# Algolzw/image-restoration-sde

Measured on AMD Instinct MI355X. Metric: restored images/sec at 256x256, 100-step IR-SDE reverse sampler, higher is better.
Workload: dtype f32; 1 GPU; IR-SDE deraining ConditionalUNet nf=64 depth=4, reverse_sde, batch=16/GPU 256x256, T=100 (BASELINE.json configs[1]); compute_dtype=fp32, global_batch=16

## Files before the change

image_restoration_sde_amd/_lib.py:

```python
import ctypes
import os
import subprocess
import threading

_HERE = os.path.dirname(os.path.abspath(__file__))
LIB_PATH = os.environ.get("IRSDE_LIB_PATH") or os.path.join(_HERE, "libirsde_hip.so")
CSRC = os.path.join(_HERE, "csrc")

MODE = {"sde": 0, "ode": 1, "posterior": 2, "dsde_sde": 3, "dsde_ode": 4}
COEF_STRIDE = 12
FLAG_KEEP_ACTIVATIONS = 1
FLAG_NAIVE_CONV = 2
FLAG_NO_WINOGRAD = 4
FLAG_NO_WINOGRAD_F43 = 8
FLAG_UNCOND_FULLATTN = 16
FLAG_BF16 = 32
FLAG_NAF_INTRO_SKIP = 64
FLAG_BF16_ACT = 128
FLAG_NO_FUSED_LN = 256
FLAG_NAF_LENS = 512
FLAG_FP16 = 1024
FLAG_NO_WINOGRAD_FUSED = 2048
FLAG_NO_FUSED_ATTN = 4096
FLAG_NO_NAF_CHAIN = 8192
FLAG_SPLIT_BF16X2 = 16384
FLAG_SPLIT_F16X2 = 32768
FLAG_NAF_STEREO = 65536
FLAG_NAF_UNCOND = 131072
FLAG_UNET_STEREO = 262144
FLAG_F16_ACT = 524288
SAMPLE_GRAPH = 1
SAMPLE_PROFILE = 2

SYMBOLS = [
    "irsde_last_error", "irsde_version", "irsde_create", "irsde_create_nafnet", "irsde_destroy", "irsde_num_weights",
    "irsde_weight_name", "irsde_weight_shape", "irsde_load_weight", "irsde_finalize_weights",
    "irsde_set_schedule", "irsde_unet_forward", "irsde_sample", "irsde_sde_step", "irsde_philox_normal",
    "irsde_get_profile", "irsde_debug_tap", "irsde_work_model", "irsde_debug_conv", "irsde_plan_describe", "irsde_bench_conv", "irsde_op_profile", "irsde_debug_split_gemm", "irsde_bench_naf_chain", "irsde_debug_force_subbatches", "irsde_debug_force_chain_groups", "irsde_debug_scam", "irsde_debug_scam_full",
    "irsde_debug_naf_gate_sca", "irsde_debug_tlsc", "irsde_debug_ln_film", "irsde_debug_naf_lnconv", "irsde_debug_naf_chain", "irsde_debug_naf_chain_split_order",
    "irsde_debug_full_attention16",
    "irsde_eval_metrics", "irsde_tensor2img",
    "irsde_set_lens_info", "irsde_nafnet_set_local_pool", "irsde_create_latent_unet", "irsde_latent_shapes", "irsde_latent_encode", "irsde_latent_decode", "irsde_latent_hidden",
]


class IrsdeLibraryError(RuntimeError):
    pass


class IrsdeError(RuntimeError):
    pass


# ... 55 lines not shown
                                 c.c_int, c.c_int, P, P, c.c_int]
    lib.irsde_sde_step.argtypes = [c.c_int, c.c_int, P, P, P, P, P, c.c_uint64, c.c_uint64, c.c_int, c.c_int,
                                   c.c_int, c.c_int, P]
    lib.irsde_philox_normal.argtypes = [P, c.c_int, c.c_int, c.c_int, c.c_uint64, c.c_uint64, P]
    lib.irsde_get_profile.argtypes = [P, c.POINTER(c.c_double)]
    lib.irsde_debug_tap.argtypes = [P, c.c_char_p, P, c.POINTER(c.c_int64)]
    lib.irsde_work_model.argtypes = [P, c.c_int, c.c_int, c.c_int, c.POINTER(c.c_double)]
    lib.irsde_debug_conv.argtypes = [P, c.c_int, P, c.c_int, c.c_int, c.c_int, c.c_int, c.c_int, P, c.c_int, c.c_int,
                                     c.c_int, c.c_int, c.c_int, P, P, c.c_int, c.c_int, P, P, c.c_int, c.c_int, P]
    lib.irsde_plan_describe.argtypes = [P, c.c_int, c.c_int, c.c_int, c.c_char_p, c.c_int]
    lib.irsde_op_profile.argtypes = [P, c.c_char_p, c.c_int]
    lib.irsde_bench_conv.argtypes = [c.c_int] * 11 + [c.POINTER(c.c_double)]
    lib.irsde_bench_naf_chain.argtypes = [c.c_int] * 4 + [c.POINTER(c.c_double)]
    lib.irsde_debug_force_subbatches.argtypes = [c.c_int]
    lib.irsde_debug_force_chain_groups.argtypes = [c.c_int]
    lib.irsde_debug_scam.argtypes = [P, c.c_int, c.c_int, c.c_int, c.c_int] + [P] * 12 + [P, P]
    lib.irsde_debug_scam_full.argtypes = [P, c.c_int, c.c_int, c.c_int, c.c_int] + [P] * 12 + [P, P]
    lib.irsde_debug_naf_gate_sca.argtypes = [P, c.c_int, c.c_int, c.c_int, c.c_int] + [P] * 8
    lib.irsde_debug_tlsc.argtypes = [P] + [c.c_int] * 6 + [P] * 4
    lib.irsde_debug_ln_film.argtypes = [P, c.c_int64, c.c_int, c.c_int64, P, P, P, c.c_int, P, P]
    lib.irsde_debug_naf_lnconv.argtypes = [c.c_int, P, c.c_int64, c.c_int, c.c_int, c.c_int64, P, P, P, c.c_int, P, P, P, c.c_int, P, P, P, P, P]
    lib.irsde_debug_naf_chain.argtypes = [P, P, c.c_int, c.c_int] + [P] * 16 + [P, c.c_int, c.c_int, P, c.c_int, c.c_int, c.c_int, P]
    lib.irsde_debug_naf_chain_split_order.argtypes = [c.c_int, c.c_int, c.POINTER(c.c_int), c.c_int64]
    lib.irsde_debug_full_attention16.argtypes = [P, c.c_int, c.c_int, P, P]
    lib.irsde_debug_split_gemm.argtypes = [P, P, P, c.c_int, c.c_int, c.c_int, c.c_int, c.c_int, P]
    lib.irsde_eval_metrics.argtypes = [P, P, c.c_int, c.c_int, c.c_int, c.c_int, c.c_int, c.POINTER(c.c_double), P]
    lib.irsde_tensor2img.argtypes = [P, P, c.c_int, c.c_int, c.c_int, c.c_int, P]
    lib.irsde_set_lens_info.argtypes = [P, c.POINTER(c.c_float), c.c_int]
    lib.irsde_nafnet_set_local_pool.argtypes = [P, c.c_int, c.c_int, c.c_int, c.c_int]
    lib.irsde_create_latent_unet.argtypes = [c.POINTER(LatentConfig), c.POINTER(P)]
# ... 51 lines not shown
```

image_restoration_sde_amd/csrc/common.h:

```cpp
#pragma once
#include <hip/hip_runtime.h>
#include <cstdint>
#include <cstdio>
#include <cstdlib>
#include <stdexcept>
#include <string>
#include <vector>

namespace irsde {

struct HipError : std::runtime_error {
    using std::runtime_error::runtime_error;
};
struct HipOutOfMemory : HipError {
    using HipError::HipError;
};

inline int tuning_env_int(const char* name, int dflt) {
    static const bool on = [] { const char* t = getenv("IRSDE_TUNING"); return t && atoi(t) == 1; }();
    if (!on) return dflt;
    const char* v = getenv(name);
    return v ? atoi(v) : dflt;
}

// ... 60 lines not shown
    int v_f16 = 0;
    float v_scale = 1.f;
    int v_pairs = 0;
    const float* M = nullptr;
    int Cout = 0;
    float* out = nullptr;
    int out_stride = 0;
    const float* bias = nullptr;
    const float* film = nullptr;
    int film_bstride = 0;
    int silu = 0;
    const float* res = nullptr;
    int res_stride = 0;
};
void launch_wino_input(const WinoParams& p, hipStream_t s);
struct SplitGemmArgs {
    const unsigned short* a = nullptr;
    const unsigned short* b = nullptr;
    float* out = nullptr;
    long long plA = 0, plB = 0, pA = 0, pB = 0, pO = 0;
    int M = 0, N = 0, K = 0, lda = 0, ldc = 0;
    float out_scale = 1.f;
    int n_inner = 1;
    int nblk_n = 0;
};
void gemm_split_global_init();
int gemm_split_inner(int M, int N, int ncomp);
void launch_gemm_split_pairs(const SplitGemmArgs& a, int ncomp, hipStream_t s, int abl = 0, bool f16 = false);
void launch_split_pairs(const float* in, unsigned short* out, size_t rows, int K, hipStream_t s, bool f16 = false,
                        float scale = 1.0f);
// ... 183 lines not shown
```

image_restoration_sde_amd/csrc/engine.h:

```cpp
#pragma once
#include <algorithm>
#include <cmath>
#include <cstring>
#include <functional>
#include <map>
#include <memory>
#include <mutex>
#include <string>
#include <vector>

#include "../../include/irsde_hip.h"
#include "common.h"

namespace irsde {

constexpr int kWinoFusedMaxCin = 256, kWinoFusedMaxCout = 256;
inline long long wino_fused_min_tiles() { return tuning_env_int("IRSDE_WINO_FUSED_MINT", 4096); }
inline bool wino_fused64_enabled() { return tuning_env_int("IRSDE_WINO_FUSED64", 1) != 0; }
inline bool wino_fused64_pair_enabled() { return tuning_env_int("IRSDE_WINO_FUSED64_PAIR", 1) != 0; }
inline int wino_fused64_max_cin() { return tuning_env_int("IRSDE_WINO_FUSED64_MAXCIN", 512); }
inline int wino_fused64_max_cout() { return tuning_env_int("IRSDE_WINO_FUSED64_MAXCOUT", 512); }
inline long long wino_fused64_min_tiles() { return tuning_env_int("IRSDE_WINO_FUSED64_MINT", 1024); }
inline int wino_fused64t_mode() { return tuning_env_int("IRSDE_WINO_FUSED64T", 1); }
inline bool naf_lnconv_enabled() { return tuning_env_int("IRSDE_NAF_LNCONV", 1) != 0; }
inline int naf_chain_split_mode() { return tuning_env_int("IRSDE_NAF_CHAIN_SPLIT", 0); }

inline int wino_min_c(int tile) {
    return tuning_env_int(tile == 4 ? "IRSDE_WINO4_MINC" : "IRSDE_WINO2_MINC", tile == 4 ? 64 : 256);
}

struct DeviceScope {
    int prev = -1;
    explicit DeviceScope(int dev) {
        if (hipGetDevice(&prev) != hipSuccess) prev = -1;
        if (prev != dev) IRSDE_HIP_CHECK(hipSetDevice(dev));
        else prev = -1;
    }
    ~DeviceScope() {
        if (prev >= 0) (void)hipSetDevice(prev);
    }
// ... 7 lines not shown
    bool loaded = false;
};

struct ConvW {
    float* w = nullptr;
    float* bias = nullptr;
    int Cout = 0, Cin = 0, KH = 1, KW = 1;
    float* wino_u2 = nullptr;
    float* wino_u4 = nullptr;
    float* wino_uf = nullptr;
    float* wino_uf64 = nullptr;
    unsigned short* wino_uf64p = nullptr;
    float wino_uf64p_scale = 1.f;
    unsigned short* wino_up = nullptr;
    float wino_up_scale = 1.f;
};
struct ResW {
    ConvW b1, b2, res;
    bool has_res = false;
    float* mlp_w = nullptr;
    float* mlp_b = nullptr;
    int film_off = 0;
    int Cout = 0;
};
struct ScamW {
    int c = 0;
    float *gl = nullptr, *gr = nullptr;
    ConvW l, r;
    float *beta = nullptr, *gamma = nullptr;
};
// ... 48 lines not shown
    const int Ctot = d.C0 + d.C1;
    const int TH = d.Ho / tile, TW = d.Wo / tile, T = d.B * TH * TW;
    const int ncomp = (tile + 2) * (tile + 2);
    w.in.tile = tile;
    w.in.in0 = d.in0; w.in.in1 = d.in1; w.in.C0 = d.C0; w.in.C1 = d.C1; w.in.Hin = d.Hin; w.in.Win = d.Win;
    w.in.in_shift = d.in_shift; w.in.B = d.B; w.in.TH = TH; w.in.TW = TW; w.in.T = T; w.in.V = V;
    w.out = w.in;
    w.out.M = Mb; w.out.Cout = d.Cout; w.out.out = d.out; w.out.out_stride = d.out_stride; w.out.bias = d.bias;
    w.out.film = d.film; w.out.film_bstride = d.film_bstride; w.out.silu = d.silu; w.out.res = d.res;
    w.out.res_stride = d.res_stride;
    ConvParams& g = w.gemm;
    g.in0 = V; g.C0 = Ctot; g.pix0 = Ctot; g.Hin = 1; g.Win = T; g.w = U; g.Cout = d.Cout;
    g.KH = g.KW = 1; g.stride = 1; g.pad_y = g.pad_x = 0; g.B = 1; g.Ho = 1; g.Wo = T;
    g.out = Mb; g.out_stride = d.Cout; g.zeros = d.zeros;
    g.nz = ncomp; g.z_in = (long long)T * Ctot; g.z_w = (long long)d.Cout * Ctot; g.z_out = (long long)T * d.Cout;
    return w;
}
struct WinoSplitPlan {
    WinoParams in, out;
    SplitGemmArgs gemm;
    int nplanes = 0;
    bool f16 = false;
};
inline WinoSplitPlan make_wino_split(const ConvParams& d, const unsigned short* Us, unsigned short* Vs, float* Mb, int nplanes) {
    const WinoPlan w = make_wino(d, nullptr, nullptr, Mb, 4);
    WinoSplitPlan sp;
    sp.in = w.in; sp.out = w.out; sp.nplanes = nplanes;
    const int Ctot = d.C0 + d.C1;
    const long long T = w.in.T;
    sp.in.Vs = Vs; sp.in.nplanes = nplanes; sp.in.v_plane = 36ll * T * Ctot;
// ... 296 lines not shown
```

image_restoration_sde_amd/csrc/engine_debug.hip:

```cpp
#include "engine.h"
#include "../../include/irsde_hip_debug.h"

using namespace irsde;

namespace irsde {
namespace {

struct Scratch {
    hipStream_t s;
    std::vector<void*> bufs;
    explicit Scratch(hipStream_t s_) : s(s_) {}
    ~Scratch() {
        (void)hipStreamSynchronize(s);
        for (void* p : bufs) (void)hipFree(p);
    }
    Scratch(const Scratch&) = delete;
    Scratch& operator=(const Scratch&) = delete;
    template <class T> T* alloc(size_t n) {
        void* p = nullptr;
        IRSDE_HIP_CHECK(hipMalloc(&p, n * sizeof(T)));
        bufs.push_back(p);
        return static_cast<T*>(p);
    }
    float* upload(const float* host, size_t n) {
// ... 30 lines not shown
    for (int i = 0; i < iters; ++i) run();
    IRSDE_HIP_CHECK(hipEventRecord(ev.e1, s));
    IRSDE_HIP_CHECK(hipStreamSynchronize(s));
    float ms = 0.f;
    IRSDE_HIP_CHECK(hipEventElapsedTime(&ms, ev.e0, ev.e1));
    return ms / iters;
}

struct VariantScope {
    explicit VariantScope(int v) { conv_set_variant(v); }
    ~VariantScope() { conv_set_variant(0); }
};

bool code_in(const std::initializer_list<int>& codes, int c) { return std::find(codes.begin(), codes.end(), c) != codes.end(); }
bool debug_conv_code_known(int c) {
    return code_in({0, 1, 2, 3, 4, 5, 12, 13, 22, 23, 33, 34, 35, 36, 37, 42, 43, 44, 45, 46, 47, 55, 56, 62, 63, 204, 260, 261, 262, 263}, c) ||
           code_in({100, 103, 105, 106, 107, 150, 160, 161, 162, 163, 165, 166, 167, 170, 171, 172, 173}, c);
}
bool bench_conv_variant_known(int v) {
    return code_in({0, 3, 5, 6, 7, 50, 60, 61, 62, 63, 64, 65, 66, 67, 70, 71, 72, 73}, v) ||
           code_in({80, 81, 82, 412, 413, 421, 422, 423, 430, 431, 432, 434, 435, 460, 461, 462, 465, 467, 468, 469, 480, 481, 482}, v) ||
           code_in({2001, 2002, 2004, 4650, 4651, 4652, 4653}, v) ||
           (v >= 83 && v <= 82 + 255) ||
           (v >= 472 && v <= 476);
}

struct ScamHookArgs {
    const float* x;
    float* out;
    const float *norm_l_g, *norm_r_g, *l_proj1_w, *l_proj1_b, *r_proj1_w, *r_proj1_b, *l_proj2_w, *l_proj2_b, *r_proj2_w, *r_proj2_b, *beta, *gamma;
};
// ... 260 lines not shown
        p.Hin = Hin; p.Win = Win; p.in_shift = in_shift;
        p.w = dw; p.Cout = Cout; p.KH = KH; p.KW = KW; p.stride = stride; p.pad_y = pad; p.pad_x = pad;
        p.B = B;
        p.Ho = ((Hin << in_shift) + 2 * pad - KH) / stride + 1;
        p.Wo = ((Win << in_shift) + 2 * pad - KW) / stride + 1;
        p.out = out; p.out_stride = Cout; p.bias = db; p.film = film; p.film_bstride = film_bstride; p.silu = silu;
        p.res = res; p.res_stride = Cout;
        float* dz = mem.alloc<float>(256);
        IRSDE_HIP_CHECK(hipMemset(dz, 0, 1024));
        p.zeros = dz;
        const int wino_tile = (naive == 2 || naive == 12 || naive == 22) ? 2 : (naive == 3 || naive == 13 || naive == 23) ? 4 : 0;
        if (splits > 1 && naive != 1 && !wino_tile) {
            p.splits = splits;
            p.partial = mem.alloc<float>((size_t)splits * B * p.Ho * p.Wo * Cout);
        }
        if (naive == 44 || naive == 45) {
            const bool f16 = naive == 44;
            if (!wino_shape_ok(p, 4) || Cin % 32) throw HipError("debug_conv: shape not eligible for the pair GEMM");
            std::vector<float> U((size_t)36 * Cout * Cin);
            wino_transform_weights(pk.data(), Cout, Cin, U.data(), 4);
            const float us = f16 ? pow2_scale_into_512(U.data(), U.size()) : 1.f;
            const long long T = (long long)B * (p.Ho / 4) * (p.Wo / 4);
            float* dU = mem.upload(U);
            unsigned short* dUp = mem.alloc<unsigned short>(2 * U.size());
            unsigned short* dVp = mem.alloc<unsigned short>((size_t)36 * T * Cin * 2);
            float* dM = mem.alloc<float>((size_t)36 * T * Cout);
            launch_split_pairs(dU, dUp, (size_t)36 * Cout, Cin, s, f16, us);
            const WinoSplitPlan sp = make_wino_pairs(p, dUp, dVp, dM, f16, us);
            launch_wino_input(sp.in, s);
            launch_gemm_split_pairs(sp.gemm, 36, s, 0, f16);
            launch_wino_output(sp.out, s);
// ... 130 lines not shown
        g.a = da; g.b = db; g.out = C;
        g.plA = (long long)na; g.plB = (long long)nb;
        g.pA = (long long)M * K; g.pB = (long long)N * K; g.pO = (long long)M * N;
        g.M = M; g.N = N; g.K = K; g.lda = K; g.ldc = N;
        g.n_inner = gemm_split_inner(M, N, ncomp);
        launch_gemm_split(g, nplanes, ncomp, s);
        IRSDE_HIP_CHECK(hipStreamSynchronize(s));
    });
}

int irsde_debug_force_chain_groups(int g) {
    set_force_chain_groups(g == 1 || g == 2 || g == 4 ? g : 0);
    return IRSDE_OK;
}

int irsde_debug_force_subbatches(int n) {
    set_force_subbatches(n < 0 ? 0 : n);
    return IRSDE_OK;
}

int irsde_bench_naf_chain(int variant, int nblocks, int B, int iters, double* ms_out) {
    return guard([&] {
        if (!ms_out || nblocks < 1 || nblocks > 64 || B < 1 || iters < 1) throw HipError("bench_naf_chain: bad argument");
        const int G = variant == 22 ? 2 : (variant == 24 || variant == 25 || variant == 26) ? 4 : 1;
#ifdef IRSDE_PROBES
        if (variant != 0 && variant != 1 && variant != 11 && G == 1) throw HipError("bench_naf_chain: bad variant");
#else
        if (variant != 0 && variant != 1 && G == 1) throw HipError("bench_naf_chain: variant 11 is a measurement twin (make PROBES=1)");
#endif
        conv_global_init();
// ... 325 lines not shown
```

image_restoration_sde_amd/csrc/engine_plan.hip:

```cpp
#include "engine.h"
#include <atomic>

using namespace irsde;

namespace irsde {

struct Builder {
    irsde_engine* e;
    Plan* pl;
    bool reuse;
    bool naive;
    int film_bstride;
    int b0 = 0;
    const float* film_base() const { return film_of(e, pl) + (size_t)b0 * film_bstride; }
    const float* cam_base() const { return e->cam_cur + (size_t)b0 * e->cam_row; }
    const float* fused_ln_g = nullptr;

    bool act_bf16() const { return (e->cfg.flags & IRSDE_FLAG_BF16_ACT) != 0; }
    bool act_f16() const { return (e->cfg.flags & IRSDE_FLAG_F16_ACT) != 0; }
    Tensor talloc(int B, int H, int W, int C, int force_f32 = 0) {
        Tensor t;
        t.B = B; t.H = H; t.W = W; t.C = C;
        t.bf16 = act_bf16() && !force_f32;
        t.f16 = act_f16() && !force_f32;
// ... 72 lines not shown
        const int Hv = in0.H << in_shift, Wv = in0.W << in_shift;
        p.B = in0.B;
        p.Ho = (Hv + 2 * pad - w.KH) / stride + 1;
        p.Wo = (Wv + 2 * pad - w.KW) / stride + 1;
        const int ostr = out_stride ? out_stride : w.Cout;
        Tensor out = talloc(p.B, p.Ho, p.Wo, ostr, out_stride != 0);
        p.out = out.p; p.out_stride = ostr;
        p.in_bf16 = in0.bf16; p.out_bf16 = out.bf16;
        p.ln_g = fused_ln_g;
        if ((in1 && in1->bf16 != in0.bf16) || (res && res->bf16 != out.bf16)) throw HipError("conv: mixed activation storage types");
        p.bias = w.bias;
        p.film = film; p.film_bstride = film ? film_bstride : 0;
        p.silu = silu;
        if (res) { p.res = res->p; p.res_stride = res->C; }
        if (!naive) {
            if (w.wino_up && wino_shape_ok(p, 4) && push_wino(p, w.wino_u4, 4, w.wino_up, w.wino_up_scale)) return out;
            if (w.wino_uf64p && push_wino_fused(p, reinterpret_cast<const float*>(w.wino_uf64p), true, w.wino_uf64p_scale)) return out;
            if (w.wino_uf64 && push_wino_fused(p, w.wino_uf64, true)) return out;
            if (w.wino_uf && push_wino_fused(p, w.wino_uf, false)) return out;
            if (w.wino_u4 && wino_shape_ok(p, 4) && push_wino(p, w.wino_u4, 4)) return out;
            if (w.wino_u2 && wino_shape_ok(p, 2) && push_wino(p, w.wino_u2, 2)) return out;
        }
        push_conv(p);
        return out;
    }

    bool push_wino_fused(const ConvParams& d, const float* Uf, bool k64, float pair_uscale = 0.f) {
        ConvParams dd = d;
        dd.zeros = e->zeros;
        if (pair_uscale != 0.f) dd.pair_scale = 1.0f / (kWinoFused64PairVScale * pair_uscale);
// ... 36 lines not shown
            const size_t b0 = (size_t)i * dd.B;
            q.in0 = dd.in0 + b0 * dd.Hin * dd.Win * dd.pix0;
            if (dd.in1) q.in1 = dd.in1 + b0 * dd.Hin * dd.Win * dd.pix1;
            q.out = dd.out + b0 * dd.Ho * dd.Wo * dd.out_stride;
            if (dd.res) q.res = dd.res + b0 * dd.Ho * dd.Wo * dd.res_stride;
            if (dd.film && dd.film_bstride) q.film = dd.film + b0 * dd.film_bstride;
            slices.push_back(q);
        }
        if (use_t)
            op.fn = [slices, Uf](hipStream_t s) { for (const auto& q : slices) launch_wino_fused64t(q, Uf, s, 0); };
        else if (k64)
            op.fn = [slices, Uf, pair](hipStream_t s) { for (const auto& q : slices) launch_wino_fused64(q, Uf, s, pair ? 4 : 0); };
        else
            op.fn = [slices, Uf](hipStream_t s) { for (const auto& q : slices) launch_wino_fused(q, Uf, s); };
        push_op(std::move(op));
        return true;
    }

    bool push_wino(const ConvParams& d, const float* U, int tile, const unsigned short* Up = nullptr, float up_scale = 1.f) {
        const int Ctot = d.C0 + d.C1;
        const int ncomp = (tile + 2) * (tile + 2);
        const long long T = (long long)d.B * (d.Ho / tile) * (d.Wo / tile);
        const long long gemm_blocks = ncomp * ((T + 127) / 128) * ((d.Cout + 127) / 128);
        if (gemm_blocks < 256) return false;
        ConvParams dd = d;
        dd.zeros = e->zeros;
        if (Up && (T < 256 || d.Cout < 256 || (unsigned long long)T * Ctot * 4ull >= 0xffffffffull)) return false;
        float* V = pl->alloc((size_t)ncomp * T * Ctot, true);
        float* Mb = pl->alloc((size_t)ncomp * T * d.Cout, true);
        WinoPlan wp = make_wino(dd, U, V, Mb, tile);
// ... 646 lines not shown
    if (stereo) {
        float* pred = pl->alloc((size_t)pl->B * pl->Hp * pl->Wp * pl->pred_stride, false);
        const float* src = pr.p;
        const int Bp = pl->B, ic = e->naf_ic, Hp = pl->Hp, Wp = pl->Wp, is = oe.out_stride, os = pl->pred_stride;
        b.push_other(OP_OTHER, [=](hipStream_t s) { launch_stereo_pack_pred(src, pred, Bp, ic, Hp, Wp, is, os, s); });
        pl->net_ops.back().desc = "stereo_pack_pred";
        pl->pred = pred;
        return;
    }
    pl->pred = pr.p;
}

static std::atomic<int> g_force_chain_groups{0};
void set_force_chain_groups(int g) { g_force_chain_groups.store(g, std::memory_order_relaxed); }
int forced_chain_groups() { return g_force_chain_groups.load(std::memory_order_relaxed); }
static std::atomic<int> g_force_subbatches{0};
void set_force_subbatches(int n) { g_force_subbatches.store(n, std::memory_order_relaxed); }
int naf_subbatches(const irsde_engine* e, int B, int H, int W) {
    if (e->arch == 2 || stereo_engine(e) || (e->cfg.flags & (IRSDE_FLAG_NAIVE_CONV | IRSDE_FLAG_KEEP_ACTIVATIONS))) return 1;
    int n = g_force_subbatches.load(std::memory_order_relaxed);
    if (n <= 0) {
        static const int env = tuning_env_int("IRSDE_SUBBATCHES", 0);
        n = env;
    }
    if (n <= 0 && e->arch != 1) n = 1;
    if (n <= 0) {
        bool chain = false;
        const int nlev = (int)e->naf_enc.size(), ps = 1 << nlev;
        const int Hp = (H + ps - 1) / ps * ps, Wp = (W + ps - 1) / ps * ps;
        if ((e->cfg.flags & IRSDE_FLAG_FP16) && !(e->cfg.flags & (IRSDE_FLAG_NO_NAF_CHAIN | IRSDE_FLAG_F16_ACT)))
// ... 298 lines not shown
```

image_restoration_sde_amd/csrc/engine_weights.hip:

```cpp
#include "engine.h"
#include <cmath>

using namespace irsde;

namespace irsde {

void finalize_common(irsde_engine* e);
void add_w(irsde_engine* e, const std::string& name, std::vector<int64_t> shape) {
    e->names.push_back(name);
    HostTensor t;
    t.shape = std::move(shape);
    e->host[name] = std::move(t);
}
void inv_resblock(irsde_engine* e, const std::string& p, int ci, int co) {
    const int td = e->time_dim;
    add_w(e, p + "mlp.1.weight", {2 * co, td});
    add_w(e, p + "mlp.1.bias", {2 * co});
    add_w(e, p + "block1.proj.weight", {co, ci, 3, 3});
    add_w(e, p + "block2.proj.weight", {co, co, 3, 3});
    if (ci != co) add_w(e, p + "res_conv.weight", {co, ci, 1, 1});
}
void inv_attn(irsde_engine* e, const std::string& p, int c) {
    add_w(e, p + "fn.norm.g", {1, c, 1, 1});
    add_w(e, p + "fn.fn.to_qkv.weight", {384, c, 1, 1});
// ... 60 lines not shown
    } else {
        inv_attn(e, "mid_attn.", mid);
    }
    inv_resblock(e, "mid_block2.", mid, mid);
    inv_resblock(e, "final_res_block.", 2 * nf, nf);
    add_w(e, "final_conv.weight", {vout, nf, 3, 3});
    add_w(e, "final_conv.bias", {vout});
}

const HostTensor& need(irsde_engine* e, const std::string& n) {
    auto it = e->host.find(n);
    if (it == e->host.end() || !it->second.loaded) throw HipError("missing weight: " + n);
    return it->second;
}

ConvW pack_conv(irsde_engine* e, const std::string& wname, const std::string& bname) {
    const HostTensor& t = need(e, wname);
    const int O = (int)t.shape[0], I = (int)t.shape[1], KH = (int)t.shape[2], KW = (int)t.shape[3];
    std::vector<float> p((size_t)O * KH * KW * I);
    for (int o = 0; o < O; ++o)
        for (int i = 0; i < I; ++i)
            for (int ky = 0; ky < KH; ++ky)
                for (int kx = 0; kx < KW; ++kx)
                    p[(((size_t)o * KH + ky) * KW + kx) * I + i] = t.data[(((size_t)o * I + i) * KH + ky) * KW + kx];
    ConvW c;
    c.w = e->upload(p);
    c.Cout = O; c.Cin = I; c.KH = KH; c.KW = KW;
    if (!bname.empty()) c.bias = e->upload(need(e, bname).data);
    if (KH == 3 && KW == 3 && I % 32 == 0 && !(e->cfg.flags & (IRSDE_FLAG_NO_WINOGRAD | IRSDE_FLAG_BF16))) {
        for (int tile : {2, 4}) {
            if (tile == 4 && (e->cfg.flags & IRSDE_FLAG_NO_WINOGRAD_F43)) continue;
            if (I < wino_min_c(tile) || O < wino_min_c(tile)) continue;
            std::vector<float> U((size_t)(tile + 2) * (tile + 2) * O * I);
            wino_transform_weights(p.data(), O, I, U.data(), tile);
            (tile == 4 ? c.wino_u4 : c.wino_u2) = e->upload(U);
            if (tile == 4 && (e->cfg.flags & (IRSDE_FLAG_SPLIT_BF16X2 | IRSDE_FLAG_SPLIT_F16X2)) && I >= split_min_cin()) {
                unsigned short* up = nullptr;
                IRSDE_HIP_CHECK(hipMalloc(&up, U.size() * 4));
                e->dev_allocs.push_back(reinterpret_cast<float*>(up));
                const bool f16 = (e->cfg.flags & IRSDE_FLAG_SPLIT_F16X2) != 0;
                if (f16) c.wino_up_scale = pow2_scale_into_512(U.data(), U.size());
                launch_split_pairs(c.wino_u4, up, (size_t)36 * O, I, e->stream, f16, c.wino_up_scale);
                IRSDE_HIP_CHECK(hipStreamSynchronize(e->stream));
// ... 563 lines not shown
        a.qkv = pack_conv(e, "mid_attn.fn.fn.to_qkv.weight", "");
        a.out = pack_conv(e, "mid_attn.fn.fn.to_out.weight", "mid_attn.fn.fn.to_out.bias");
        a.C = a.out.Cout;
        e->mid_attn = a;
    } else {
        e->mid_attn = pack_attn(e, "mid_attn.");
    }
    e->mid2 = pack_res(e, "mid_block2.");
    for (int j = 0; j < depth; ++j) {
        const std::string u = "ups." + std::to_string(j) + ".";
        e->up_res.push_back(pack_res(e, u + "0."));
        e->up_res.push_back(pack_res(e, u + "1."));
        e->up_attn.push_back(pack_attn(e, u + "2."));
        if (stereo) e->up_scam.push_back(pack_scam(e, u + "3."));
        if (j != depth - 1)
            e->up_conv.push_back(pack_conv(e, u + ci + ".1.weight", u + ci + ".1.bias"));
        else
            e->up_conv.push_back(pack_conv(e, u + ci + ".weight", ""));
    }
    e->final_res = pack_res(e, "final_res_block.");
    e->final_conv = pack_conv(e, "final_conv.weight", "final_conv.bias");

    e->all_res.clear();
    for (auto& r : e->down_res) e->all_res.push_back(&r);
    e->all_res.push_back(&e->mid1);
    e->all_res.push_back(&e->mid2);
    for (auto& r : e->up_res) e->all_res.push_back(&r);
    e->all_res.push_back(&e->final_res);
    int off = 0;
    for (ResW* r : e->all_res) {
        r->film_off = off;
// ... 67 lines not shown
```

image_restoration_sde_amd/csrc/wino.hip:

```cpp
#include "common.h"

namespace irsde {
namespace {

__device__ __forceinline__ float4 operator+(float4 a, float4 b) { return make_float4(a.x + b.x, a.y + b.y, a.z + b.z, a.w + b.w); }
__device__ __forceinline__ float4 operator-(float4 a, float4 b) { return make_float4(a.x - b.x, a.y - b.y, a.z - b.z, a.w - b.w); }
__device__ __forceinline__ float4 operator*(float s, float4 a) { return make_float4(s * a.x, s * a.y, s * a.z, s * a.w); }
__device__ __forceinline__ float silu1(float v) { return v / (1.0f + expf(-v)); }
template <typename V> struct VecOps;
template <> struct VecOps<float4> {
    static constexpr int N = 4;
    static __device__ __forceinline__ float4 zero() { return make_float4(0.f, 0.f, 0.f, 0.f); }
    static __device__ __forceinline__ float4 one() { return make_float4(1.f, 1.f, 1.f, 1.f); }
    static __device__ __forceinline__ float4 mad(float4 v, float4 a, float4 b) { return make_float4(v.x * a.x + b.x, v.y * a.y + b.y, v.z * a.z + b.z, v.w * a.w + b.w); }
    static __device__ __forceinline__ float4 silu(float4 v) { return make_float4(silu1(v.x), silu1(v.y), silu1(v.z), silu1(v.w)); }
};
template <> struct VecOps<float> {
    static constexpr int N = 1;
    static __device__ __forceinline__ float zero() { return 0.f; }
    static __device__ __forceinline__ float one() { return 1.f; }
    static __device__ __forceinline__ float mad(float v, float a, float b) { return v * a + b; }
    static __device__ __forceinline__ float silu(float v) { return silu1(v); }
};

// ... 221 lines not shown
    for (int i = 0; i < TILE; ++i) {
        V y[TILE];
        at_apply<TILE, V>(u[i], y);
#pragma unroll
        for (int j = 0; j < TILE; ++j) {
            const size_t pixel = ((size_t)b * Ho + TILE * ty + i) * Wo + TILE * tx + j;
            V v = y[j] + bias;
            if (p.film) v = VecOps<V>::mad(v, sc, sh);
            if (p.silu) v = VecOps<V>::silu(v);
            if (p.res) v = v + *reinterpret_cast<const V*>(p.res + pixel * p.res_stride + n);
            *reinterpret_cast<V*>(p.out + pixel * p.out_stride + n) = v;
        }
    }
}

}

static int wino_vec() {
    static const int v = tuning_env_int("IRSDE_WINO_VEC", 4);
    return v;
}

void launch_wino_input(const WinoParams& p, hipStream_t s) {
    if (p.Vs) {
        if (p.tile != 4 || (p.nplanes != 2 && p.nplanes != 3) || (p.C0 % 4) || (p.C1 % 4)) throw HipError("wino_input (split): F(4x4,3x3), 2 or 3 planes");
        const long long tot = (long long)p.T * ((p.C0 + p.C1) / 4);
        const dim3 gr((unsigned)((tot + 255) / 256));
        if (p.v_pairs) {
            if (p.nplanes != 2 || (p.C0 + p.C1) % 32) throw HipError("wino_input (pairs): two planes, channels a multiple of 32");
            if (p.v_f16) hipLaunchKernelGGL((wino_input_split_kernel<2, true, true>), gr, dim3(256), 0, s, p);
// ... 58 lines not shown
```

include/irsde_hip.h:

```cpp
#ifndef IRSDE_HIP_H
#define IRSDE_HIP_H

#include <stdint.h>

#ifdef __cplusplus
extern "C" {
#endif

typedef struct irsde_engine irsde_engine;

enum {
    IRSDE_OK = 0,
    IRSDE_ERR_INVALID = -1,
    IRSDE_ERR_HIP = -2,
    IRSDE_ERR_STATE = -3,
    IRSDE_ERR_WEIGHT = -4
};

enum { IRSDE_MODE_SDE = 0, IRSDE_MODE_ODE = 1, IRSDE_MODE_POSTERIOR = 2,
       IRSDE_MODE_DSDE_SDE = 3, IRSDE_MODE_DSDE_ODE = 4 };

enum {
    IRSDE_FLAG_KEEP_ACTIVATIONS = 1,
    IRSDE_FLAG_NAIVE_CONV = 2,
// ... 2 lines not shown
    IRSDE_FLAG_BF16 = 32,
    IRSDE_FLAG_BF16_ACT = 128,
    IRSDE_FLAG_NO_FUSED_LN = 256,
    IRSDE_FLAG_NAF_LENS = 512,
    IRSDE_FLAG_NAF_INTRO_SKIP = 64,
    IRSDE_FLAG_FP16 = 1024,
    IRSDE_FLAG_NO_WINOGRAD_FUSED = 2048,
    IRSDE_FLAG_NO_FUSED_ATTN = 4096,
    IRSDE_FLAG_SPLIT_BF16X2 = 16384,
    IRSDE_FLAG_SPLIT_F16X2 = 32768,
    IRSDE_FLAG_NO_NAF_CHAIN = 8192,
    IRSDE_FLAG_NAF_STEREO = 65536,
    IRSDE_FLAG_NAF_UNCOND = 131072,
    IRSDE_FLAG_UNET_STEREO = 262144,
    IRSDE_FLAG_F16_ACT = 524288,
    IRSDE_FLAG_NO_WINOGRAD_F43 = 8
};
enum {
    IRSDE_SAMPLE_GRAPH = 1,
    IRSDE_SAMPLE_PROFILE = 2
};

typedef struct irsde_config {
    int32_t in_nc;
    int32_t out_nc;
    int32_t nf;
    int32_t depth;
    int32_t device;
    int32_t flags;
} irsde_config;
// ... 87 lines not shown
```

include/irsde_hip_debug.h:

```cpp
#ifndef IRSDE_HIP_DEBUG_H
#define IRSDE_HIP_DEBUG_H

#include "irsde_hip.h"

#ifdef __cplusplus
extern "C" {
#endif

int irsde_debug_conv(const float* in0, int C0, const float* in1, int C1, int B, int Hin, int Win, int in_shift,
                     const float* w_oihw, int Cout, int KH, int KW, int stride, int pad, const float* bias,
                     const float* film, int film_bstride, int silu, const float* res, float* out, int naive,
                     int splits, void* stream);

int irsde_debug_split_gemm(const float* A, const float* B, float* C, int M, int N, int K, int ncomp, int nplanes, void* stream);

int irsde_bench_conv(int variant, int B, int H, int W, int Cin, int Cout, int K, int stride, int up, int epi, int iters,
                     double* ms_out);
int irsde_bench_naf_chain(int variant, int nblocks, int B, int iters, double* ms_out);
int irsde_debug_force_subbatches(int n);
int irsde_debug_force_chain_groups(int g);

int irsde_debug_scam(const float* x, int B_pairs, int H, int W, int C, const float* norm_l_g, const float* norm_r_g, const float* l_proj1_w,
                     const float* l_proj1_b, const float* r_proj1_w, const float* r_proj1_b, const float* l_proj2_w, const float* l_proj2_b,
                     const float* r_proj2_w, const float* r_proj2_b, const float* beta, const float* gamma, float* out, void* stream);

int irsde_debug_naf_gate_sca(const float* u, int B, int H, int W, int c, const float* conv2_w, const float* conv2_b, const float* sca_w, const float* sca_b,
                             float* gated_out, float* mean_out, float* s_out, void* stream);
int irsde_debug_tlsc(const float* g, int B, int h, int w, int c, int k1, int k2, float* pooled_out, const float* scale_map, float* scaled_out, void* stream);
int irsde_debug_ln_film(const float* x, long long M, int C, long long ppi, const float* g, const float* fscale, const float* fshift, int film_bstride,
                        float* out, void* stream);
int irsde_debug_naf_lnconv(int mode, const float* x, long long M, int c, int Cout, long long ppi, const float* g, const float* fscale, const float* fshift,
                           int film_bstride, const float* w, const float* bias, const float* gate_film, int gate_film_bstride, const float* in_scale,
                           const float* ch_scale, const float* res, float* out, void* stream);

int irsde_debug_naf_chain(const float* x, float* out, int B, int nblocks, const float* norm1_g, const float* conv1_w, const float* conv1_b, const float* conv2_w,
// ... 16 lines not shown
```

Measured before the change: 4.262 images/s.

## Add polyphase Winograd F(4,2) path for strided-down and upsample convolutions

Adds a Winograd F(4x4,2x2) path that splits 4x4 stride-2 downsampling convs and nearest-upsample-plus-3x3 convs into four 2x2 polyphase sub-kernels. Each is computed through 5x5 input and output transforms around a batched per-component GEMM. The goal is to cut multiply count and direct-conv cost for resampling layers. It is enabled by default behind size heuristics (enough GEMM blocks and FLOPs; upsample only when Cin>=512), with a flag and env/debug overrides to disable it. It adds extra workspace buffers and precomputed transformed weights, and larger Winograd tiles bring some fp32 rounding risk.

```diff
diff --git a/image_restoration_sde_amd/_lib.py b/image_restoration_sde_amd/_lib.py
--- a/image_restoration_sde_amd/_lib.py
+++ b/image_restoration_sde_amd/_lib.py
@@ -29,6 +29,7 @@
 FLAG_NAF_UNCOND = 131072
 FLAG_UNET_STEREO = 262144
 FLAG_F16_ACT = 524288
+FLAG_NO_WINO_POLY = 1048576
 SAMPLE_GRAPH = 1
 SAMPLE_PROFILE = 2
 
@@ -36,7 +37,7 @@
     "irsde_last_error", "irsde_version", "irsde_create", "irsde_create_nafnet", "irsde_destroy", "irsde_num_weights",
     "irsde_weight_name", "irsde_weight_shape", "irsde_load_weight", "irsde_finalize_weights",
     "irsde_set_schedule", "irsde_unet_forward", "irsde_sample", "irsde_sde_step", "irsde_philox_normal",
-    "irsde_get_profile", "irsde_debug_tap", "irsde_work_model", "irsde_debug_conv", "irsde_plan_describe", "irsde_bench_conv", "irsde_op_profile", "irsde_debug_split_gemm", "irsde_bench_naf_chain", "irsde_debug_force_subbatches", "irsde_debug_force_chain_groups", "irsde_debug_scam", "irsde_debug_scam_full",
+    "irsde_get_profile", "irsde_debug_tap", "irsde_work_model", "irsde_debug_conv", "irsde_plan_describe", "irsde_bench_conv", "irsde_op_profile", "irsde_debug_split_gemm", "irsde_bench_naf_chain", "irsde_debug_force_subbatches", "irsde_debug_force_chain_groups", "irsde_debug_force_wino_poly", "irsde_debug_scam", "irsde_debug_scam_full",
     "irsde_debug_naf_gate_sca", "irsde_debug_tlsc", "irsde_debug_ln_film", "irsde_debug_naf_lnconv", "irsde_debug_naf_chain", "irsde_debug_naf_chain_split_order",
     "irsde_debug_full_attention16",
     "irsde_eval_metrics", "irsde_tensor2img",
@@ -122,6 +123,7 @@
     lib.irsde_bench_naf_chain.argtypes = [c.c_int] * 4 + [c.POINTER(c.c_double)]
     lib.irsde_debug_force_subbatches.argtypes = [c.c_int]
     lib.irsde_debug_force_chain_groups.argtypes = [c.c_int]
+    lib.irsde_debug_force_wino_poly.argtypes = [c.c_int]
     lib.irsde_debug_scam.argtypes = [P, c.c_int, c.c_int, c.c_int, c.c_int] + [P] * 12 + [P, P]
     lib.irsde_debug_scam_full.argtypes = [P, c.c_int, c.c_int, c.c_int, c.c_int] + [P] * 12 + [P, P]
     lib.irsde_debug_naf_gate_sca.argtypes = [P, c.c_int, c.c_int, c.c_int, c.c_int] + [P] * 8
diff --git a/image_restoration_sde_amd/csrc/common.h b/image_restoration_sde_amd/csrc/common.h
--- a/image_restoration_sde_amd/csrc/common.h
+++ b/image_restoration_sde_amd/csrc/common.h
@@ -98,6 +98,21 @@
     int res_stride = 0;
 };
 void launch_wino_input(const WinoParams& p, hipStream_t s);
+struct WinoPolyParams {
+    int up = 0;
+    const float* in = nullptr;
+    int C = 0, Hin = 0, Win = 0;
+    int B = 0, TH = 0, TW = 0, T = 0;
+    float* V = nullptr;
+    const float* M = nullptr;
+    int Cout = 0, Ho = 0, Wo = 0;
+    float* out = nullptr;
+    int out_stride = 0;
+    const float* bias = nullptr;
+};
+void launch_wino_poly_input(const WinoPolyParams& p, hipStream_t s);
+void launch_wino_poly_output(const WinoPolyParams& p, hipStream_t s);
+void wino_poly_transform_weights(const float* w_packed, int Cout, int Cin, float* U, int up);
 struct SplitGemmArgs {
     const unsigned short* a = nullptr;
     const unsigned short* b = nullptr;
diff --git a/image_restoration_sde_amd/csrc/engine.h b/image_restoration_sde_amd/csrc/engine.h
--- a/image_restoration_sde_amd/csrc/engine.h
+++ b/image_restoration_sde_amd/csrc/engine.h
@@ -24,6 +24,11 @@
 inline int wino_fused64t_mode() { return tuning_env_int("IRSDE_WINO_FUSED64T", 1); }
 inline bool naf_lnconv_enabled() { return tuning_env_int("IRSDE_NAF_LNCONV", 1) != 0; }
 inline int naf_chain_split_mode() { return tuning_env_int("IRSDE_NAF_CHAIN_SPLIT", 0); }
+
+int wino_poly_mode();
+void set_force_wino_poly(int mode);
+constexpr int kWinoPolyUpMinCin = 512;
+inline bool wino_poly_wants_weights(int mode, bool up, int Cin) { return mode >= 2 || (mode == 1 && (!up || Cin >= kWinoPolyUpMinCin)); }
 
 inline int wino_min_c(int tile) {
     return tuning_env_int(tile == 4 ? "IRSDE_WINO4_MINC" : "IRSDE_WINO2_MINC", tile == 4 ? 64 : 256);
@@ -61,6 +66,7 @@
     float wino_uf64p_scale = 1.f;
     unsigned short* wino_up = nullptr;
     float wino_up_scale = 1.f;
+    float* wino_poly = nullptr;
 };
 struct ResW {
     ConvW b1, b2, res;
@@ -139,6 +145,38 @@
     g.KH = g.KW = 1; g.stride = 1; g.pad_y = g.pad_x = 0; g.B = 1; g.Ho = 1; g.Wo = T;
     g.out = Mb; g.out_stride = d.Cout; g.zeros = d.zeros;
     g.nz = ncomp; g.z_in = (long long)T * Ctot; g.z_w = (long long)d.Cout * Ctot; g.z_out = (long long)T * d.Cout;
+    return w;
+}
+inline bool wino_poly_down_shape(const ConvParams& d) {
+    return d.KH == 4 && d.KW == 4 && d.stride == 2 && d.pad_y == 1 && d.pad_x == 1 && !d.in_shift && d.Hin >= 2 && d.Win >= 2;
+}
+inline bool wino_poly_up_shape(const ConvParams& d) { return d.KH == 3 && d.KW == 3 && d.stride == 1 && d.pad_y == 1 && d.pad_x == 1 && d.in_shift == 1; }
+inline bool wino_poly_eligible(const ConvParams& d) {
+    return (wino_poly_down_shape(d) || wino_poly_up_shape(d)) && !d.in1 && !d.C1 && d.C0 % 32 == 0 && d.pix0 == d.C0 && d.Cout % 4 == 0 && d.out_stride % 4 == 0 &&
+           !d.film && !d.silu && !d.res && !d.ln_g && !d.ch_scale && !d.in_scale && !d.gate && !d.shuffle && !d.in_bf16 && !d.out_bf16 && !d.in_f16 && !d.out_f16;
+}
+struct WinoPolyPlan {
+    WinoPolyParams in, out;
+    ConvParams gemm;
+    int ncomp = 0;
+    long long T = 0;
+    int K = 0;
+};
+inline WinoPolyPlan make_wino_poly(const ConvParams& d, const float* U, float* V, float* Mb) {
+    WinoPolyPlan w;
+    const int up = d.in_shift ? 1 : 0;
+    WinoPolyParams& q = w.in;
+    q.up = up; q.in = d.in0; q.C = d.C0; q.Hin = d.Hin; q.Win = d.Win; q.B = d.B;
+    q.Ho = d.Ho; q.Wo = d.Wo;
+    q.TH = ((up ? d.Hin : d.Ho) + 3) / 4; q.TW = ((up ? d.Win : d.Wo) + 3) / 4; q.T = d.B * q.TH * q.TW;
+    q.V = V; q.M = Mb; q.Cout = d.Cout; q.out = d.out; q.out_stride = d.out_stride; q.bias = d.bias;
+    w.out = q;
+    w.ncomp = up ? 100 : 25; w.T = q.T; w.K = up ? d.C0 : 4 * d.C0;
+    ConvParams& g = w.gemm;
+    g.in0 = V; g.C0 = w.K; g.pix0 = w.K; g.Hin = 1; g.Win = q.T; g.w = U; g.Cout = d.Cout;
+    g.KH = g.KW = 1; g.stride = 1; g.pad_y = g.pad_x = 0; g.B = 1; g.Ho = 1; g.Wo = q.T;
+    g.out = Mb; g.out_stride = d.Cout; g.zeros = d.zeros;
+    g.nz = w.ncomp; g.z_in = (long long)q.T * w.K; g.z_w = (long long)d.Cout * w.K; g.z_out = (long long)q.T * d.Cout;
     return w;
 }
 struct WinoSplitPlan {
diff --git a/image_restoration_sde_amd/csrc/engine_debug.hip b/image_restoration_sde_amd/csrc/engine_debug.hip
--- a/image_restoration_sde_amd/csrc/engine_debug.hip
+++ b/image_restoration_sde_amd/csrc/engine_debug.hip
@@ -68,7 +68,7 @@
 
 bool code_in(const std::initializer_list<int>& codes, int c) { return std::find(codes.begin(), codes.end(), c) != codes.end(); }
 bool debug_conv_code_known(int c) {
-    return code_in({0, 1, 2, 3, 4, 5, 12, 13, 22, 23, 33, 34, 35, 36, 37, 42, 43, 44, 45, 46, 47, 55, 56, 62, 63, 204, 260, 261, 262, 263}, c) ||
+    return code_in({0, 1, 2, 3, 4, 5, 12, 13, 22, 23, 24, 25, 33, 34, 35, 36, 37, 42, 43, 44, 45, 46, 47, 55, 56, 62, 63, 204, 260, 261, 262, 263}, c) ||
            code_in({100, 103, 105, 106, 107, 150, 160, 161, 162, 163, 165, 166, 167, 170, 171, 172, 173}, c);
 }
 bool bench_conv_variant_known(int v) {
@@ -359,7 +359,22 @@
             p.splits = splits;
             p.partial = mem.alloc<float>((size_t)splits * B * p.Ho * p.Wo * Cout);
         }
-        if (naive == 44 || naive == 45) {
+        if (naive == 24 || naive == 25) {
+            if (!(naive == 24 ? wino_poly_down_shape(p) : wino_poly_up_shape(p)) || !wino_poly_eligible(p) || splits > 1)
+                throw HipError(naive == 24 ? "debug_conv: selector 24 runs a 4x4 stride-2 pad-1 convolution (single source, channels a multiple of 32, bias only)"
+                                           : "debug_conv: selector 25 runs a 3x3 stride-1 pad-1 convolution with in_shift = 1 (single source, channels a multiple of 32, bias only)");
+            const int up = naive == 25;
+            std::vector<float> U((size_t)100 * Cout * Cin);
+            wino_poly_transform_weights(pk.data(), Cout, Cin, U.data(), up);
+            float* dU = mem.upload(U);
+            WinoPolyPlan wp = make_wino_poly(p, dU, nullptr, nullptr);
+            float* dV = mem.alloc<float>((size_t)wp.ncomp * wp.T * wp.K);
+            float* dM = mem.alloc<float>((size_t)wp.ncomp * wp.T * Cout);
+            wp = make_wino_poly(p, dU, dV, dM);
+            launch_wino_poly_input(wp.in, s);
+            launch_conv(wp.gemm, s);
+            launch_wino_poly_output(wp.out, s);
+        } else if (naive == 44 || naive == 45) {
             const bool f16 = naive == 44;
             if (!wino_shape_ok(p, 4) || Cin % 32) throw HipError("debug_conv: shape not eligible for the pair GEMM");
             std::vector<float> U((size_t)36 * Cout * Cin);
@@ -520,6 +535,11 @@
     return IRSDE_OK;
 }
 
+int irsde_debug_force_wino_poly(int mode) {
+    set_force_wino_poly(mode >= 0 && mode <= 2 ? mode : -1);
+    return IRSDE_OK;
+}
+
 int irsde_debug_force_subbatches(int n) {
     set_force_subbatches(n < 0 ? 0 : n);
     return IRSDE_OK;
diff --git a/image_restoration_sde_amd/csrc/engine_plan.hip b/image_restoration_sde_amd/csrc/engine_plan.hip
--- a/image_restoration_sde_amd/csrc/engine_plan.hip
+++ b/image_restoration_sde_amd/csrc/engine_plan.hip
@@ -110,6 +110,7 @@
         p.silu = silu;
         if (res) { p.res = res->p; p.res_stride = res->C; }
         if (!naive) {
+            if (w.wino_poly && push_wino_poly(p, w.wino_poly)) return out;
             if (w.wino_up && wino_shape_ok(p, 4) && push_wino(p, w.wino_u4, 4, w.wino_up, w.wino_up_scale)) return out;
             if (w.wino_uf64p && push_wino_fused(p, reinterpret_cast<const float*>(w.wino_uf64p), true, w.wino_uf64p_scale)) return out;
             if (w.wino_uf64 && push_wino_fused(p, w.wino_uf64, true)) return out;
@@ -176,6 +177,56 @@
         else
             op.fn = [slices, Uf](hipStream_t s) { for (const auto& q : slices) launch_wino_fused(q, Uf, s); };
         push_op(std::move(op));
+        return true;
+    }
+
+    bool push_wino_poly(const ConvParams& d, const float* U) {
+        const int mode = wino_poly_mode();
+        if (mode <= 0 || !wino_poly_eligible(d)) return false;
+        ConvParams dd = d;
+        dd.zeros = e->zeros;
+        WinoPolyPlan wp = make_wino_poly(dd, U, nullptr, nullptr);
+        const long long T = wp.T;
+        const long long gemm_blocks = wp.ncomp * ((T + 127) / 128) * ((d.Cout + 127) / 128);
+        const double exec_flops = wp.ncomp * 2.0 * (double)T * wp.K * d.Cout;
+        if (mode == 1 && (gemm_blocks < 2ll * device_cu_count() || exec_flops < 2e10)) return false;
+        if ((unsigned long long)T * std::max(wp.K, d.Cout) * 4ull >= 0x7fffffffull) return false;
+        float* V = pl->alloc((size_t)wp.ncomp * T * wp.K, true);
+        float* Mb = pl->alloc((size_t)wp.ncomp * T * d.Cout, true);
+        wp = make_wino_poly(dd, U, V, Mb);
+        const char* what = wp.in.up ? "up" : "down";
+        {
+            Op op;
+            op.kind = OP_WINO;
+            op.desc = std::string("wino_poly_input(") + what + ") T=" + std::to_string(T) + " C=" + std::to_string(d.C0);
+            const WinoPolyParams ip = wp.in;
+            op.fn = [ip](hipStream_t s) { launch_wino_poly_input(ip, s); };
+            pl->net_ops.push_back(std::move(op));
+        }
+        {
+            Op op;
+            op.kind = OP_CONV;
+            op.flops = conv_flops(d);
+            op.exec_flops = exec_flops;
+            op.bytes = 4.0 * (double)d.B * d.Hin * d.Win * d.C0 + 4.0 * (double)d.B * d.Ho * d.Wo * d.Cout + 4.0 * (double)d.KH * d.KW * d.Cout * d.C0;
+            char buf[256];
+            snprintf(buf, sizeof buf, "conv(winograd F4x2 poly %s gemm x%d) T=%lld Cout=%d Cin=%d K=%d flops=%.4g exec=%.4g", what, wp.ncomp, T, d.Cout, d.C0, wp.K,
+                     op.flops, op.exec_flops);
+            op.desc = buf;
+            const ConvParams g = wp.gemm;
+            op.fn = [g](hipStream_t s) { launch_conv(g, s); };
+            push_op(std::move(op));
+        }
+        {
+            Op op;
+            op.kind = OP_WINO;
+            op.desc = std::string("wino_poly_output(") + what + ") T=" + std::to_string(T) + " Cout=" + std::to_string(d.Cout);
+            const WinoPolyParams oparm = wp.out;
+            op.fn = [oparm](hipStream_t s) { launch_wino_poly_output(oparm, s); };
+            pl->net_ops.push_back(std::move(op));
+        }
+        pl->release(V);
+        pl->release(Mb);
         return true;
     }
 
@@ -852,6 +903,12 @@
 static std::atomic<int> g_force_chain_groups{0};
 void set_force_chain_groups(int g) { g_force_chain_groups.store(g, std::memory_order_relaxed); }
 int forced_chain_groups() { return g_force_chain_groups.load(std::memory_order_relaxed); }
+static std::atomic<int> g_force_wino_poly{-1};
+void set_force_wino_poly(int mode) { g_force_wino_poly.store(mode, std::memory_order_relaxed); }
+int wino_poly_mode() {
+    const int f = g_force_wino_poly.load(std::memory_order_relaxed);
+    return f >= 0 ? f : tuning_env_int("IRSDE_WINO_POLY", 1);
+}
 static std::atomic<int> g_force_subbatches{0};
 void set_force_subbatches(int n) { g_force_subbatches.store(n, std::memory_order_relaxed); }
 int naf_subbatches(const irsde_engine* e, int B, int H, int W) {
diff --git a/image_restoration_sde_amd/csrc/engine_weights.hip b/image_restoration_sde_amd/csrc/engine_weights.hip
--- a/image_restoration_sde_amd/csrc/engine_weights.hip
+++ b/image_restoration_sde_amd/csrc/engine_weights.hip
@@ -98,7 +98,7 @@
     return it->second;
 }
 
-ConvW pack_conv(irsde_engine* e, const std::string& wname, const std::string& bname) {
+ConvW pack_conv(irsde_engine* e, const std::string& wname, const std::string& bname, int resample = 0) {
     const HostTensor& t = need(e, wname);
     const int O = (int)t.shape[0], I = (int)t.shape[1], KH = (int)t.shape[2], KW = (int)t.shape[3];
     std::vector<float> p((size_t)O * KH * KW * I);
@@ -111,6 +111,15 @@
     c.w = e->upload(p);
     c.Cout = O; c.Cin = I; c.KH = KH; c.KW = KW;
     if (!bname.empty()) c.bias = e->upload(need(e, bname).data);
+    constexpr int kNotExactF32 = IRSDE_FLAG_NO_WINOGRAD | IRSDE_FLAG_NAIVE_CONV | IRSDE_FLAG_BF16 | IRSDE_FLAG_BF16_ACT | IRSDE_FLAG_FP16 | IRSDE_FLAG_F16_ACT |
+                                 IRSDE_FLAG_SPLIT_BF16X2 | IRSDE_FLAG_SPLIT_F16X2 | IRSDE_FLAG_NO_WINO_POLY;
+    const bool poly_up = resample && KH == 3 && KW == 3, poly_down = KH == 4 && KW == 4;
+    if ((poly_up || poly_down) && I % 32 == 0 && O % 4 == 0 && !bname.empty() && !(e->cfg.flags & kNotExactF32) &&
+        wino_poly_wants_weights(wino_poly_mode(), poly_up, I)) {
+        std::vector<float> U((size_t)(poly_up ? 100 : 25 * 4) * O * I);
+        wino_poly_transform_weights(p.data(), O, I, U.data(), poly_up ? 1 : 0);
+        c.wino_poly = e->upload(U);
+    }
     if (KH == 3 && KW == 3 && I % 32 == 0 && !(e->cfg.flags & (IRSDE_FLAG_NO_WINOGRAD | IRSDE_FLAG_BF16))) {
         for (int tile : {2, 4}) {
             if (tile == 4 && (e->cfg.flags & IRSDE_FLAG_NO_WINOGRAD_F43)) continue;
@@ -704,7 +713,7 @@
         e->up_attn.push_back(pack_attn(e, u + "2."));
         if (stereo) e->up_scam.push_back(pack_scam(e, u + "3."));
         if (j != depth - 1)
-            e->up_conv.push_back(pack_conv(e, u + ci + ".1.weight", u + ci + ".1.bias"));
+            e->up_conv.push_back(pack_conv(e, u + ci + ".1.weight", u + ci + ".1.bias", 1));
         else
             e->up_conv.push_back(pack_conv(e, u + ci + ".weight", ""));
     }
diff --git a/image_restoration_sde_amd/csrc/wino.hip b/image_restoration_sde_amd/csrc/wino.hip
--- a/image_restoration_sde_amd/csrc/wino.hip
+++ b/image_restoration_sde_amd/csrc/wino.hip
@@ -259,6 +259,193 @@
     }
 }
 
+__device__ __forceinline__ void bt5_apply(const float4* d, float4* t) {
+    t[0] = 2.0f * (d[0] - d[2]) + (d[3] - d[1]);
+    t[1] = (d[3] - d[2]) - 2.0f * d[1];
+    t[2] = 2.0f * d[1] - 3.0f * d[2] + d[3];
+    t[3] = d[3] - d[1];
+    t[4] = 2.0f * (d[1] - d[3]) + (d[4] - d[2]);
+}
+__device__ __forceinline__ void at5_apply(const float4* m, float4* y) {
+    const float4 s12 = m[1] + m[2], d12 = m[1] - m[2];
+    y[0] = m[0] + s12 + m[3];
+    y[1] = d12 + 2.0f * m[3];
+    y[2] = s12 + 4.0f * m[3];
+    y[3] = d12 + 8.0f * m[3] + m[4];
+}
+
+template <bool UP>
+__global__ __launch_bounds__(256) void wino_poly_input_kernel(const WinoPolyParams p) {
+    const int C4 = p.C / 4;
+    const long long idx = (long long)blockIdx.x * blockDim.x + threadIdx.x;
+    const long long total = (long long)p.T * 4 * C4;
+    if (idx >= total) return;
+    const int c = (int)(idx % C4) * 4;
+    const long long i1 = idx / C4;
+    const int ph = (int)(i1 & 3);
+    const int t = (int)(i1 >> 2);
+    const int tx = t % p.TW;
+    const int t1 = t / p.TW;
+    const int ty = t1 % p.TH;
+    const int b = t1 / p.TH;
+    constexpr int STEP = UP ? 1 : 2;
+    const int y0 = 4 * STEP * ty - 1 + (ph >> 1), x0 = 4 * STEP * tx - 1 + (ph & 1);
+    const float* src = p.in + c;
+    float4 w[5][5];
+    {
+        float4 d[5][5];
+#pragma unroll
+        for (int r = 0; r < 5; ++r) {
+            const int iy = y0 + STEP * r;
+#pragma unroll
+            for (int s = 0; s < 5; ++s) {
+                const int ix = x0 + STEP * s;
+                const bool ok = (unsigned)iy < (unsigned)p.Hin && (unsigned)ix < (unsigned)p.Win;
+                const size_t pixel = (size_t)b * p.Hin * p.Win + (size_t)(ok ? iy : 0) * p.Win + (ok ? ix : 0);
+                const float4 v = *reinterpret_cast<const float4*>(src + pixel * p.C);
+                d[r][s] = ok ? v : make_float4(0.f, 0.f, 0.f, 0.f);
+            }
+        }
+#pragma unroll
+        for (int s = 0; s < 5; ++s) {
+            float4 col[5], tc[5];
+#pragma unroll
+            for (int r = 0; r < 5; ++r) col[r] = d[r][s];
+            bt5_apply(col, tc);
+#pragma unroll
+            for (int r = 0; r < 5; ++r) w[r][s] = tc[r];
+        }
+    }
+    const size_t K = UP ? (size_t)p.C : (size_t)4 * p.C;
+    const size_t kstride = (size_t)p.T * K;
+    float* vp = UP ? p.V + (size_t)ph * 25 * kstride + (size_t)t * K + c : p.V + (size_t)t * K + (size_t)ph * p.C + c;
+#pragma unroll
+    for (int r = 0; r < 5; ++r) {
+        float4 o[5];
+        bt5_apply(w[r], o);
+#pragma unroll
+        for (int s = 0; s < 5; ++s) *reinterpret_cast<float4*>(vp + (size_t)(r * 5 + s) * kstride) = o[s];
+    }
+}
+
+template <bool UP>
+__global__ __launch_bounds__(256) void wino_poly_output_kernel(const WinoPolyParams p) {
+    const int N4 = p.Cout / 4;
+    const long long idx = (long long)blockIdx.x * blockDim.x + threadIdx.x;
+    const long long total = (long long)p.T * (UP ? 4 : 1) * N4;
+    if (idx >= total) return;
+    const int n = (int)(idx % N4) * 4;
+    const long long i1 = idx / N4;
+    const int ph = UP ? (int)(i1 & 3) : 0;
+    const int t = UP ? (int)(i1 >> 2) : (int)i1;
+    const int tx = t % p.TW;
+    const int t1 = t / p.TW;
+    const int ty = t1 % p.TH;
+    const int b = t1 / p.TH;
+    const size_t kstride = (size_t)p.T * p.Cout;
+    const float* mp = p.M + (size_t)ph * 25 * kstride + (size_t)t * p.Cout + n;
+    float4 u[4][5];
+    {
+        float4 m[5][5];
+#pragma unroll
+        for (int r = 0; r < 5; ++r)
+#pragma unroll
+            for (int s = 0; s < 5; ++s) m[r][s] = *reinterpret_cast<const float4*>(mp + (size_t)(r * 5 + s) * kstride);
+#pragma unroll
+        for (int s = 0; s < 5; ++s) {
+            float4 col[5], yc[4];
+#pragma unroll
+            for (int r = 0; r < 5; ++r) col[r] = m[r][s];
+            at5_apply(col, yc);
+#pragma unroll
+            for (int i = 0; i < 4; ++i) u[i][s] = yc[i];
+        }
+    }
+    float4 bias = make_float4(0.f, 0.f, 0.f, 0.f);
+    if (p.bias) bias = *reinterpret_cast<const float4*>(p.bias + n);
+    const int LH = UP ? p.Hin : p.Ho, LW = UP ? p.Win : p.Wo;
+#pragma unroll
+    for (int i = 0; i < 4; ++i) {
+        float4 y[4];
+        at5_apply(u[i], y);
+        const int ly = 4 * ty + i;
+#pragma unroll
+        for (int j = 0; j < 4; ++j) {
+            const int lx = 4 * tx + j;
+            if (ly >= LH || lx >= LW) continue;
+            const int oy = UP ? 2 * ly + (ph >> 1) : ly, ox = UP ? 2 * lx + (ph & 1) : lx;
+            const size_t pixel = ((size_t)b * p.Ho + oy) * p.Wo + ox;
+            *reinterpret_cast<float4*>(p.out + pixel * p.out_stride + n) = y[j] + bias;
+        }
+    }
+}
+
+}
+
+static void wino_poly_check(const WinoPolyParams& p, bool output) {
+    const int LH = p.up ? p.Hin : p.Ho, LW = p.up ? p.Win : p.Wo;
+    if (p.C <= 0 || p.C % 4 || p.B <= 0 || p.Hin <= 0 || p.Win <= 0 || p.TH != (LH + 3) / 4 || p.TW != (LW + 3) / 4 || p.T != p.B * p.TH * p.TW)
+        throw HipError("wino_poly: inconsistent tiling");
+    if (p.up ? (p.Ho != 2 * p.Hin || p.Wo != 2 * p.Win) : (p.Ho != (p.Hin - 2) / 2 + 1 || p.Wo != (p.Win - 2) / 2 + 1 || p.Hin < 2 || p.Win < 2))
+        throw HipError("wino_poly: output size does not belong to the input size");
+    if (output && (p.Cout <= 0 || p.Cout % 4 || p.out_stride % 4 || p.out_stride < p.Cout)) throw HipError("wino_poly_output: channels must be multiples of 4");
+}
+
+void launch_wino_poly_input(const WinoPolyParams& p, hipStream_t s) {
+    wino_poly_check(p, false);
+    const long long total = (long long)p.T * p.C;
+    const dim3 grid((unsigned)((total + 255) / 256));
+    if (p.up) hipLaunchKernelGGL((wino_poly_input_kernel<true>), grid, dim3(256), 0, s, p);
+    else hipLaunchKernelGGL((wino_poly_input_kernel<false>), grid, dim3(256), 0, s, p);
+    IRSDE_HIP_CHECK(hipGetLastError());
+}
+
+void launch_wino_poly_output(const WinoPolyParams& p, hipStream_t s) {
+    wino_poly_check(p, true);
+    const long long total = (long long)p.T * (p.up ? 4 : 1) * (p.Cout / 4);
+    const dim3 grid((unsigned)((total + 255) / 256));
+    if (p.up) hipLaunchKernelGGL((wino_poly_output_kernel<true>), grid, dim3(256), 0, s, p);
+    else hipLaunchKernelGGL((wino_poly_output_kernel<false>), grid, dim3(256), 0, s, p);
+    IRSDE_HIP_CHECK(hipGetLastError());
+}
+
+void wino_poly_transform_weights(const float* w_packed, int Cout, int Cin, float* U, int up) {
+    static const double G[5][2] = {{0.5, 0.0}, {-0.5, -0.5}, {-1.0 / 6, 1.0 / 6}, {1.0 / 6, 1.0 / 3}, {0.0, 1.0}};
+    const int KW = up ? 3 : 4;
+    const size_t K = up ? (size_t)Cin : (size_t)4 * Cin;
+    const size_t kstride = (size_t)Cout * K;
+    for (int n = 0; n < Cout; ++n)
+        for (int c = 0; c < Cin; ++c) {
+            double w[4][4];
+            for (int ky = 0; ky < KW; ++ky)
+                for (int kx = 0; kx < KW; ++kx) w[ky][kx] = w_packed[(((size_t)n * KW + ky) * KW + kx) * Cin + c];
+            for (int ph = 0; ph < 4; ++ph) {
+                const int p = ph >> 1, q = ph & 1;
+                double g[2][2];
+                for (int a = 0; a < 2; ++a)
+                    for (int b = 0; b < 2; ++b) {
+                        if (!up) {
+                            g[a][b] = w[2 * a + p][2 * b + q];
+                        } else {
+                            const int y0 = p == 0 ? (a == 0 ? 0 : 1) : (a == 0 ? 0 : 2), y1 = p == 0 ? (a == 0 ? 0 : 2) : (a == 0 ? 1 : 2);
+                            const int x0 = q == 0 ? (b == 0 ? 0 : 1) : (b == 0 ? 0 : 2), x1 = q == 0 ? (b == 0 ? 0 : 2) : (b == 0 ? 1 : 2);
+                            double sum = 0.0;
+                            for (int ky = y0; ky <= y1; ++ky)
+                                for (int kx = x0; kx <= x1; ++kx) sum += w[ky][kx];
+                            g[a][b] = sum;
+                        }
+                    }
+                double tmp[5][2];
+                for (int r = 0; r < 5; ++r)
+                    for (int b = 0; b < 2; ++b) tmp[r][b] = G[r][0] * g[0][b] + G[r][1] * g[1][b];
+                for (int r = 0; r < 5; ++r)
+                    for (int s = 0; s < 5; ++s) {
+                        const float v = (float)(tmp[r][0] * G[s][0] + tmp[r][1] * G[s][1]);
+                        if (up) U[((size_t)ph * 25 + r * 5 + s) * kstride + (size_t)n * K + c] = v;
+                        else U[(size_t)(r * 5 + s) * kstride + (size_t)n * K + (size_t)ph * Cin + c] = v;
+                    }
+            }
+        }
 }
 
 static int wino_vec() {
diff --git a/include/irsde_hip.h b/include/irsde_hip.h
--- a/include/irsde_hip.h
+++ b/include/irsde_hip.h
@@ -40,6 +40,7 @@
     IRSDE_FLAG_NAF_UNCOND = 131072,
     IRSDE_FLAG_UNET_STEREO = 262144,
     IRSDE_FLAG_F16_ACT = 524288,
+    IRSDE_FLAG_NO_WINO_POLY = 1048576,
     IRSDE_FLAG_NO_WINOGRAD_F43 = 8
 };
 enum {
diff --git a/include/irsde_hip_debug.h b/include/irsde_hip_debug.h
--- a/include/irsde_hip_debug.h
+++ b/include/irsde_hip_debug.h
@@ -19,6 +19,7 @@
 int irsde_bench_naf_chain(int variant, int nblocks, int B, int iters, double* ms_out);
 int irsde_debug_force_subbatches(int n);
 int irsde_debug_force_chain_groups(int g);
+int irsde_debug_force_wino_poly(int mode);
 
 int irsde_debug_scam(const float* x, int B_pairs, int H, int W, int C, const float* norm_l_g, const float* norm_r_g, const float* l_proj1_w,
                      const float* l_proj1_b, const float* r_proj1_w, const float* r_proj1_b, const float* l_proj2_w, const float* l_proj2_b,
```

Measured after the change: 4.373 images/s (median of 6 runs). 2.6% higher.
